# kowaalczyk/reformer-tts

Measured on AMD Instinct MI355X. Metric: mel-frames/sec training step, LJSpeech-shape batch, higher is better.
Workload: dtype bf16; 1 GPU; config/baseline.yml full Reformer-TTS training step (enc 3 / dec 3 layers, d=512, LSH 8 rounds, buckets 64/128), per-GPU batch 12, text 200->256, mel 1024x80; global_batch=12, parallelism=dp1, reversible_recompute=full

## Files before the change

### reformer-tts_amd/csrc/gemm_tn.hip

```cpp
#include "rtts_common.h"
#include <atomic>

#define GT_BM 64
#define GT_PAD 64

struct GtProb {
    const bf16_t* a;
    const bf16_t* b;
    float* out;
    float* c;
    int64_t lda, ldb, ldo, ldc;
    size_t slab_stride;
    int M, N, K, split, accumulate;
    int wg_start;
    int rb_start;
};
struct GtGroup {
    GtProb p[RTTS_GEMM_TN_MAX_GROUP];
    int n;
};

template <int WN, int WK, int TN, int TK>
__global__ __launch_bounds__(64 * WN * WK) void gemm_tn_kernel(const GtGroup grp) {
    constexpr int BN = 32 * TN * WN, BK = 32 * TK * WK, NTHR = 64 * WN * WK;
    constexpr int ROWA = BN * 2 + GT_PAD, ROWB = BK * 2 + GT_PAD;
    constexpr int PA = BN / 8, PB = BK / 8;
    constexpr int ITA = GT_BM * PA / NTHR, ITB = GT_BM * PB / NTHR;
    static_assert(GT_BM * PA % NTHR == 0 && GT_BM * PB % NTHR == 0, "staging must tile");
    extern __shared__ __attribute__((aligned(16))) unsigned char smem[];
    unsigned char* As = smem;
    unsigned char* Bs = smem + 2 * GT_BM * ROWA;

    int pi = 0;
#pragma unroll
    for (int i = 1; i < RTTS_GEMM_TN_MAX_GROUP; ++i)
        if (i < grp.n && (int)blockIdx.x >= grp.p[i].wg_start) pi = i;
    const GtProb& P = grp.p[pi];
    const bf16_t* __restrict__ a = P.a;
    const bf16_t* __restrict__ b = P.b;
    float* __restrict__ out = P.out;
    const int64_t lda = P.lda, ldb = P.ldb, ldo = P.ldo;
    const int M = P.M, K = P.K, split = P.split, accumulate = P.accumulate;
    const size_t slab_stride = P.slab_stride;
    const int blk = (int)blockIdx.x - P.wg_start;

    const int tiles_k = K / BK;
    const int tile = blk / split, sp = blk % split;
    const int n0 = (tile / tiles_k) * BN, k0 = (tile % tiles_k) * BK;
    const int st_all = M / GT_BM, st_base = st_all / split, st_rem = st_all % split;
    const int nstage = st_base + (sp < st_rem ? 1 : 0);
    const int m_begin = (sp * st_base + min(sp, st_rem)) * GT_BM;

    const int tid = threadIdx.x, lane = tid & 63, wave = tid >> 6;
    const int wn = wave / WK, wk = wave % WK;
    const int hh = lane >> 5;
    const int trq = (lane & 15) >> 2, trp = lane & 3, trc = (lane >> 4) & 1;

    const int arow = tid / PA, apiece = tid % PA, brow = tid / PB, bpiece = tid % PB;
    static_assert(ITA <= 4 && ITB <= 4, "staging registers");
    uint4 ra0, ra1, ra2, ra3, rb0, rb1, rb2, rb3;
#define GT_LD(reg, base, ld, step, it, IT) \
    if constexpr ((it) < (IT)) reg = *reinterpret_cast<const uint4*>((base) + (size_t)((it) * (step)) * (ld))
#define GT_ST(reg, base, bstep, it, IT) \
    if constexpr ((it) < (IT)) *reinterpret_cast<uint4*>((base) + (it) * (bstep)) = reg
#define GT_LOAD_STAGE(stage)                                                              \
    do {                                                                                  \
        const size_t m_ = (size_t)m_begin + (size_t)(stage) * GT_BM;                      \
        const bf16_t* pa_ = a + (m_ + arow) * lda + n0 + apiece * 8;                      \
        const bf16_t* pb_ = b + (m_ + brow) * ldb + k0 + bpiece * 8;                      \
        GT_LD(ra0, pa_, lda, NTHR / PA, 0, ITA); GT_LD(ra1, pa_, lda, NTHR / PA, 1, ITA); \
        GT_LD(ra2, pa_, lda, NTHR / PA, 2, ITA); GT_LD(ra3, pa_, lda, NTHR / PA, 3, ITA); \
        GT_LD(rb0, pb_, ldb, NTHR / PB, 0, ITB); GT_LD(rb1, pb_, ldb, NTHR / PB, 1, ITB); \
        GT_LD(rb2, pb_, ldb, NTHR / PB, 2, ITB); GT_LD(rb3, pb_, ldb, NTHR / PB, 3, ITB); \
    } while (0)
#define GT_STORE_STAGE(buf)                                                               \
    do {                                                                                  \
        unsigned char* pa_ = As + ((buf) * GT_BM + arow) * ROWA + apiece * 16;            \
        unsigned char* pb_ = Bs + ((buf) * GT_BM + brow) * ROWB + bpiece * 16;            \
        GT_ST(ra0, pa_, (NTHR / PA) * ROWA, 0, ITA); GT_ST(ra1, pa_, (NTHR / PA) * ROWA, 1, ITA); \
        GT_ST(ra2, pa_, (NTHR / PA) * ROWA, 2, ITA); GT_ST(ra3, pa_, (NTHR / PA) * ROWA, 3, ITA); \
        GT_ST(rb0, pb_, (NTHR / PB) * ROWB, 0, ITB); GT_ST(rb1, pb_, (NTHR / PB) * ROWB, 1, ITB); \
        GT_ST(rb2, pb_, (NTHR / PB) * ROWB, 2, ITB); GT_ST(rb3, pb_, (NTHR / PB) * ROWB, 3, ITB); \
    } while (0)

    f32x16 acc[TN][TK];
#pragma unroll
    for (int i = 0; i < TN; ++i)
#pragma unroll
        for (int j = 0; j < TK; ++j) acc[i][j] = (f32x16){0};

    GT_LOAD_STAGE(0);
    GT_STORE_STAGE(0);
    __syncthreads();
    for (int s = 0; s < nstage; ++s) {
        const int buf = s & 1;
        if (s + 1 < nstage) GT_LOAD_STAGE(s + 1);
        const unsigned char* Ab = As + buf * GT_BM * ROWA;
        const unsigned char* Bb = Bs + buf * GT_BM * ROWB;
#define GT_FRAGS(AF, BF, ks_)                                                                   \
    do {                                                                                        \
        const int mr_ = (ks_) * 16 + 8 * hh + trq;                                              \
        _Pragma("unroll") for (int t = 0; t < TN; ++t) {                                        \
            const int ca_ = (wn * 32 * TN + t * 32 + 16 * trc + 4 * trp) * 2;                   \
            AF[t] = rtts_tr_frag(Ab + mr_ * ROWA + ca_, Ab + (mr_ + 4) * ROWA + ca_);             \
        }                                                                                       \
        _Pragma("unroll") for (int t = 0; t < TK; ++t) {                                        \
            const int cb_ = (wk * 32 * TK + t * 32 + 16 * trc + 4 * trp) * 2;                   \
            BF[t] = rtts_tr_frag(Bb + mr_ * ROWB + cb_, Bb + (mr_ + 4) * ROWB + cb_);             \
        }                                                                                       \
    } while (0)
#define GT_MFMAS(AF, BF)                                                                        \
    _Pragma("unroll") for (int i = 0; i < TN; ++i)                                              \
        _Pragma("unroll") for (int j = 0; j < TK; ++j)                                          \
            acc[i][j] = __builtin_amdgcn_mfma_f32_32x32x16_bf16(AF[i], BF[j], acc[i][j], 0, 0, 0)
        bf16x8 af0[TN], bf0[TK], af1[TN], bf1[TK];
        GT_FRAGS(af0, bf0, 0);
        GT_FRAGS(af1, bf1, 1);
        __builtin_amdgcn_sched_barrier(0);
        GT_MFMAS(af0, bf0);
        __builtin_amdgcn_sched_barrier(0);
        GT_FRAGS(af0, bf0, 2);
        __builtin_amdgcn_sched_barrier(0);
        GT_MFMAS(af1, bf1);
        __builtin_amdgcn_sched_barrier(0);
        GT_FRAGS(af1, bf1, 3);
        __builtin_amdgcn_sched_barrier(0);
        GT_MFMAS(af0, bf0);
        __builtin_amdgcn_sched_barrier(0);
        GT_MFMAS(af1, bf1);
        static_assert(GT_BM == 64, "four k-steps per stage");
        if (s + 1 < nstage) GT_STORE_STAGE(buf ^ 1);
        __syncthreads();
    }
#undef GT_LOAD_STAGE
#undef GT_STORE_STAGE
#undef GT_LD
#undef GT_ST
#undef GT_FRAGS
#undef GT_MFMAS

    float* dst = out + (split > 1 ? (size_t)sp * slab_stride : 0);
    const bool add = (split == 1) && accumulate;
#pragma unroll
    for (int i = 0; i < TN; ++i)
#pragma unroll
        for (int j = 0; j < TK; ++j) {
            const int nb = n0 + wn * 32 * TN + i * 32 + 4 * hh;
            const int kc = k0 + wk * 32 * TK + j * 32 + (lane & 31);
#pragma unroll
            for (int e = 0; e < 16; ++e) {
                float* p = dst + (size_t)(nb + (e & 3) + 8 * (e >> 2)) * ldo + kc;
                *p = add ? *p + acc[i][j][e] : acc[i][j][e];
            }
        }
}

#define GT_RS 32
#define GT_NST 4

template <int WN, int WK, int TN, int TK>
__global__ __launch_bounds__(64 * WN * WK) void gemm_tn_ring_kernel(const GtGroup grp) {
    constexpr int BN = 32 * TN * WN, BK = 32 * TK * WK, NTHR = 64 * WN * WK, NWAVE = WN * WK;
    static_assert(BN == 256 && BK == 256 && NWAVE == 8, "ring variant: 256 x 256 tile, 8 waves");
    constexpr int ROWB = 512;
    constexpr int STAGE = GT_RS * ROWB;
    extern __shared__ __attribute__((aligned(16))) unsigned char smem[];
    unsigned char* As = smem;
    unsigned char* Bs = smem + GT_NST * STAGE;

    int pi = 0;
#pragma unroll
    for (int i = 1; i < RTTS_GEMM_TN_MAX_GROUP; ++i)
        if (i < grp.n && (int)blockIdx.x >= grp.p[i].wg_start) pi = i;
    const GtProb& P = grp.p[pi];
    const bf16_t* __restrict__ a = P.a;
    const bf16_t* __restrict__ b = P.b;
    float* __restrict__ out = P.out;
    const int64_t lda = P.lda, ldb = P.ldb, ldo = P.ldo;
    const int M = P.M, K = P.K, split = P.split, accumulate = P.accumulate;
    const size_t slab_stride = P.slab_stride;
    const int blk = (int)blockIdx.x - P.wg_start;
    const int tiles_k = K / BK;
    const int tile = blk / split, sp = blk % split;
    const int n0 = (tile / tiles_k) * BN, k0 = (tile % tiles_k) * BK;
    const int st_all = M / GT_RS, st_base = st_all / split, st_rem = st_all % split;
    const int nstage = st_base + (sp < st_rem ? 1 : 0);
    const int m_begin = (sp * st_base + min(sp, st_rem)) * GT_RS;

    const int tid = threadIdx.x, lane = tid & 63, wave = __builtin_amdgcn_readfirstlane(tid >> 6);
    const int wn = wave / WK, wk = wave % WK;
    const int hh = lane >> 5;
    const int trq = (lane & 15) >> 2, trp = lane & 3, trc = (lane >> 4) & 1;

    const bf16_t* srcA[2];
    const bf16_t* srcB[2];
#pragma unroll
    for (int i = 0; i < 2; ++i) {
        const int row = 4 * wave + 2 * i + (lane >> 5);
        const int pp = lane & 31;
        const int col = ((((pp >> 2) ^ (row & 3)) << 6) + ((pp & 3) << 4)) >> 1;
        srcA[i] = a + ((size_t)m_begin + row) * lda + n0 + col;
        srcB[i] = b + ((size_t)m_begin + row) * ldb + k0 + col;
    }
#define GT_ISSUE(stage_)                                                                                              \
    do {                                                                                                              \
        const int buf_ = (stage_) % GT_NST;                                                                           \
        const size_t mo_ = (size_t)(stage_) * GT_RS;                                                                  \
        _Pragma("unroll") for (int i = 0; i < 2; ++i) {                                                               \
            __builtin_amdgcn_global_load_lds((const __attribute__((address_space(1))) void*)(srcA[i] + mo_ * lda),    \
                                             (RTTS_LDS void*)(As + buf_ * STAGE + (4 * wave + 2 * i) * ROWB), 16, 0, 0); \
            __builtin_amdgcn_global_load_lds((const __attribute__((address_space(1))) void*)(srcB[i] + mo_ * ldb),    \
                                             (RTTS_LDS void*)(Bs + buf_ * STAGE + (4 * wave + 2 * i) * ROWB), 16, 0, 0); \
        }                                                                                                             \
    } while (0)

    f32x16 acc[TN][TK];
#pragma unroll
    for (int i = 0; i < TN; ++i)
#pragma unroll
        for (int j = 0; j < TK; ++j) acc[i][j] = (f32x16){0};

    int offA[TN], offB[TK];
#pragma unroll
    for (int t = 0; t < TN; ++t) {
        const int cb = (wn * 32 * TN + t * 32 + 16 * trc + 4 * trp) * 2;
        offA[t] = (8 * hh + trq) * ROWB + ((((cb >> 6) ^ trq) << 6) | (cb & 63));
    }
#pragma unroll
    for (int t = 0; t < TK; ++t) {
        const int cb = (wk * 32 * TK + t * 32 + 16 * trc + 4 * trp) * 2;
        offB[t] = (8 * hh + trq) * ROWB + ((((cb >> 6) ^ trq) << 6) | (cb & 63));
    }

    constexpr int AHEAD = GT_NST - 1;
    static_assert(AHEAD >= 2 && AHEAD <= 4, "ring depth 3..5");
#pragma unroll
    for (int i = 0; i < AHEAD; ++i)
        if (i < nstage) GT_ISSUE(i);
    for (int s = 0; s < nstage; ++s) {
        const int later = min(AHEAD - 1, nstage - 1 - s);
        if (later >= 3) __builtin_amdgcn_s_waitcnt(0x0F7C);
        else if (later == 2) __builtin_amdgcn_s_waitcnt(0x0F78);
        else if (later == 1) __builtin_amdgcn_s_waitcnt(0x0F74);
        else __builtin_amdgcn_s_waitcnt(0x0F70);
        asm volatile("s_barrier" ::: "memory");
        if (s + AHEAD < nstage) GT_ISSUE(s + AHEAD);
        const unsigned char* Ab = As + (s % GT_NST) * STAGE;
        const unsigned char* Bb = Bs + (s % GT_NST) * STAGE;
        const uint32_t abase = (uint32_t)(uintptr_t)(RTTS_LDS unsigned char*)Ab;
        const uint32_t bbase = (uint32_t)(uintptr_t)(RTTS_LDS unsigned char*)Bb;
        short4v al[2][TN], ah[2][TN], bl[2][TK], bh[2][TK];
#define GT_TR(dst, addr, off) asm volatile("ds_read_b64_tr_b16 %0, %1 offset:%2" : "=v"(dst) : "v"(addr), "n"(off))
#pragma unroll
        for (int t = 0; t < TN; ++t) {
            const uint32_t ad = abase + offA[t];
            GT_TR(al[0][t], ad, 0);
            GT_TR(ah[0][t], ad, 4 * ROWB);
            GT_TR(al[1][t], ad, 16 * ROWB);
            GT_TR(ah[1][t], ad, 20 * ROWB);
        }
#pragma unroll
        for (int t = 0; t < TK; ++t) {
            const uint32_t ad = bbase + offB[t];
            GT_TR(bl[0][t], ad, 0);
            GT_TR(bh[0][t], ad, 4 * ROWB);
            GT_TR(bl[1][t], ad, 16 * ROWB);
            GT_TR(bh[1][t], ad, 20 * ROWB);
        }
#undef GT_TR
        static_assert(TN == 2 && TK == 4, "operand list of the wait below");
        asm volatile("s_waitcnt lgkmcnt(0)"
                     : "+v"(al[0][0]), "+v"(ah[0][0]), "+v"(al[1][0]), "+v"(ah[1][0]), "+v"(al[0][1]), "+v"(ah[0][1]), "+v"(al[1][1]),
                       "+v"(ah[1][1]), "+v"(bl[0][0]), "+v"(bh[0][0]), "+v"(bl[1][0]), "+v"(bh[1][0]), "+v"(bl[0][1]), "+v"(bh[0][1]),
                       "+v"(bl[1][1]), "+v"(bh[1][1]), "+v"(bl[0][2]), "+v"(bh[0][2]), "+v"(bl[1][2]), "+v"(bh[1][2]), "+v"(bl[0][3]),
                       "+v"(bh[0][3]), "+v"(bl[1][3]), "+v"(bh[1][3]));
        bf16x8 af0[TN], bf0[TK], af1[TN], bf1[TK];
#pragma unroll
        for (int t = 0; t < TN; ++t) {
            const short8v f0 = {al[0][t][0], al[0][t][1], al[0][t][2], al[0][t][3], ah[0][t][0], ah[0][t][1], ah[0][t][2], ah[0][t][3]};
            const short8v f1 = {al[1][t][0], al[1][t][1], al[1][t][2], al[1][t][3], ah[1][t][0], ah[1][t][1], ah[1][t][2], ah[1][t][3]};
            af0[t] = __builtin_bit_cast(bf16x8, f0);
            af1[t] = __builtin_bit_cast(bf16x8, f1);
        }
#pragma unroll
        for (int t = 0; t < TK; ++t) {
            const short8v f0 = {bl[0][t][0], bl[0][t][1], bl[0][t][2], bl[0][t][3], bh[0][t][0], bh[0][t][1], bh[0][t][2], bh[0][t][3]};
            const short8v f1 = {bl[1][t][0], bl[1][t][1], bl[1][t][2], bl[1][t][3], bh[1][t][0], bh[1][t][1], bh[1][t][2], bh[1][t][3]};
            bf0[t] = __builtin_bit_cast(bf16x8, f0);
            bf1[t] = __builtin_bit_cast(bf16x8, f1);
        }
#pragma unroll
        for (int i = 0; i < TN; ++i)
#pragma unroll
            for (int j = 0; j < TK; ++j) acc[i][j] = __builtin_amdgcn_mfma_f32_32x32x16_bf16(af0[i], bf0[j], acc[i][j], 0, 0, 0);
#pragma unroll
        for (int i = 0; i < TN; ++i)
#pragma unroll
            for (int j = 0; j < TK; ++j) acc[i][j] = __builtin_amdgcn_mfma_f32_32x32x16_bf16(af1[i], bf1[j], acc[i][j], 0, 0, 0);
    }
#undef GT_ISSUE

    float* dst = out + (split > 1 ? (size_t)sp * slab_stride : 0);
    const bool add = (split == 1) && accumulate;
#pragma unroll
    for (int i = 0; i < TN; ++i)
#pragma unroll
        for (int j = 0; j < TK; ++j) {
            const int nb = n0 + wn * 32 * TN + i * 32 + 4 * hh;
            const int kc = k0 + wk * 32 * TK + j * 32 + (lane & 31);
#pragma unroll
            for (int e = 0; e < 16; ++e) {
                float* p = dst + (size_t)(nb + (e & 3) + 8 * (e >> 2)) * ldo + kc;
                *p = add ? *p + acc[i][j][e] : acc[i][j][e];
            }
        }
}

__global__ __launch_bounds__(256) void slab_reduce_kernel(const GtGroup grp) {
    int pi = 0;
#pragma unroll
    for (int i = 1; i < RTTS_GEMM_TN_MAX_GROUP; ++i)
        if (i < grp.n && (int)blockIdx.x >= grp.p[i].rb_start) pi = i;
    const GtProb& P = grp.p[pi];
    if (P.split == 1) return;
    const size_t i4 = (size_t)((int)blockIdx.x - P.rb_start) * blockDim.x + threadIdx.x;
    const size_t total4 = P.slab_stride / 4;
    if (i4 >= total4) return;
    const size_t e = i4 * 4;
    const int n = (int)(e / P.K), k = (int)(e % P.K);
    const float* __restrict__ slabs = P.out;
    float4 s = *reinterpret_cast<const float4*>(slabs + e);
    for (int t = 1; t < P.split; ++t) {
        const float4 v = *reinterpret_cast<const float4*>(slabs + (size_t)t * P.slab_stride + e);
        s.x += v.x; s.y += v.y; s.z += v.z; s.w += v.w;
    }
    float4* dst = reinterpret_cast<float4*>(P.c + (size_t)n * P.ldc + k);
    if (P.accumulate) {
        const float4 o = *dst;
        s.x += o.x; s.y += o.y; s.z += o.z; s.w += o.w;
    }
    *dst = s;
}

template <int WN, int WK, int TN, int TK>
static int gt_launch(const GtGroup& grp, int wg, hipStream_t s) {
    constexpr int BN = 32 * TN * WN, BK = 32 * TK * WK;
    const size_t lds = 2 * GT_BM * (BN * 2 + GT_PAD) + 2 * GT_BM * (BK * 2 + GT_PAD);
    static RttsLdsState st = {};
    RTTS_ENSURE_LDS("rtts_gemm_tn", (gemm_tn_kernel<WN, WK, TN, TK>), lds, st);
    hipLaunchKernelGGL((gemm_tn_kernel<WN, WK, TN, TK>), dim3(wg), dim3(64 * WN * WK), lds, s, grp);
    return 0;
}

static bool gt_c_overlap(const rtts_gemm_tn_problem& p, const rtts_gemm_tn_problem& q) {
    const uintptr_t bp = (uintptr_t)p.c, bq = (uintptr_t)q.c;
    const uintptr_t ep = bp + ((uintptr_t)(p.N - 1) * (uintptr_t)p.ldc + (uintptr_t)p.K) * sizeof(float);
    const uintptr_t eq = bq + ((uintptr_t)(q.N - 1) * (uintptr_t)q.ldc + (uintptr_t)q.K) * sizeof(float);
    if (bq >= ep || bp >= eq) return false;
    if (p.ldc != q.ldc) return true;
    const rtts_gemm_tn_problem& lo = bp <= bq ? p : q;
    const rtts_gemm_tn_problem& hi = bp <= bq ? q : p;
    const int64_t d = (int64_t)(((uintptr_t)hi.c - (uintptr_t)lo.c) / sizeof(float));
    const int64_t r = d / lo.ldc, s = d % lo.ldc;
    if (s < lo.K) return true;
    return s + hi.K > lo.ldc && r + 1 < lo.N;
}

static std::atomic<int> g_gt_small{0};
extern "C" int rtts_debug_set_gemm_tn_tiles(int small_tiles) {
    if (small_tiles != 0 && small_tiles != 1) {
        rtts_set_error("rtts_debug_set_gemm_tn_tiles: 0 (library's pick) or 1 (128 x 128 tiles for every group) (got %d)", small_tiles);
        return -1;
    }
    g_gt_small.store(small_tiles, std::memory_order_relaxed);
    return 0;
}

extern "C" int rtts_gemm_tn_grouped(const rtts_gemm_tn_problem* problems, int n, float* slab_ws, int64_t slab_ws_floats, void* stream) {
    RTTS_ENTER(stream);
    RTTS_REQUIRE(problems && n > 0 && n <= RTTS_GEMM_TN_MAX_GROUP, "rtts_gemm_tn_grouped: 1..%d problems", RTTS_GEMM_TN_MAX_GROUP);
    GtGroup grp;
    grp.n = n;
    bool big = g_gt_small.load(std::memory_order_relaxed) == 0;
    long long flops = 0;
    for (int i = 0; i < n; ++i) {
        const rtts_gemm_tn_problem& q = problems[i];
        RTTS_REQUIRE(q.a && q.b && q.c, "rtts_gemm_tn: null pointer");
        RTTS_REQUIRE(q.N > 0 && q.K > 0 && q.M > 0 && q.N % 128 == 0 && q.K % 128 == 0 && q.M % GT_BM == 0,
                     "rtts_gemm_tn: need N %% 128 == 0, K %% 128 == 0, M %% 64 == 0 (got M=%d N=%d K=%d)", q.M, q.N, q.K);
        RTTS_REQUIRE(q.lda >= q.N && q.ldb >= q.K && q.ldc >= q.K && q.lda % 8 == 0 && q.ldb % 8 == 0 && q.ldc % 4 == 0,
                     "rtts_gemm_tn: bad leading dimensions");
        RTTS_REQUIRE((((uintptr_t)q.a | (uintptr_t)q.b | (uintptr_t)q.c) & 15) == 0, "rtts_gemm_tn: buffers must be 16-byte aligned");
        big = big && q.N % 256 == 0 && q.K % 256 == 0;
        flops += 2LL * q.M * q.N * q.K;
    }
    for (int i = 1; i < n; ++i)
        for (int j = 0; j < i; ++j)
            RTTS_REQUIRE(!gt_c_overlap(problems[j], problems[i]),
                         "rtts_gemm_tn_grouped: problems %d and %d write overlapping parts of C (launch them one after the other)", j, i);
    if (flops < 40LL * 1000000000LL) big = false;
    const int bt = big ? 256 : 128;
    int total_tiles = 0;
    for (int i = 0; i < n; ++i) total_tiles += (problems[i].N / bt) * (problems[i].K / bt);
    const int wg_target = big ? 320 : 640;
    int want = 1;
    while (total_tiles * want * 2 <= wg_target) want *= 2;
    int wg = 0, rb = 0;
    size_t slab_used = 0;
    bool any_split = false;
    for (int i = 0; i < n; ++i) {
        const rtts_gemm_tn_problem& q = problems[i];
        GtProb& P = grp.p[i];
        const int tiles = (q.N / bt) * (q.K / bt), stages = q.M / GT_BM;
        const size_t slab = (size_t)q.N * q.K;
        int split = 1;
        while (split < want && split * 2 <= stages / 4) split *= 2;
        while (split > 1 && (!slab_ws || slab_used + slab * split > (size_t)slab_ws_floats)) split /= 2;
        P.a = (const bf16_t*)q.a; P.b = (const bf16_t*)q.b; P.c = q.c;
        P.lda = q.lda; P.ldb = q.ldb; P.ldc = q.ldc;
        P.M = q.M; P.N = q.N; P.K = q.K; P.split = split; P.accumulate = q.accumulate;
        P.slab_stride = slab;
        P.wg_start = wg;
        P.rb_start = rb;
        wg += tiles * split;
        if (split > 1) {
            P.out = slab_ws + slab_used;
            P.ldo = q.K;
            slab_used += slab * split;
            rb += (int)((slab / 4 + 255) / 256);
            any_split = true;
        } else {
            P.out = q.c;
            P.ldo = q.ldc;
        }
    }
    hipStream_t s = (hipStream_t)stream;
    if (big) {
        const size_t lds = 2 * GT_NST * GT_RS * 512;
        static RttsLdsState st = {};
        RTTS_ENSURE_LDS("rtts_gemm_tn", (gemm_tn_ring_kernel<4, 2, 2, 4>), lds, st);
        hipLaunchKernelGGL((gemm_tn_ring_kernel<4, 2, 2, 4>), dim3(wg), dim3(512), lds, s, grp);
    } else if (gt_launch<2, 2, 2, 2>(grp, wg, s)) return -1;
    if (any_split) hipLaunchKernelGGL(slab_reduce_kernel, dim3(rb), dim3(256), 0, s, grp);
    RTTS_LAUNCH_CHECK("rtts_gemm_tn");
    return 0;
}

extern "C" int rtts_gemm_tn(const void* a, int64_t lda, const void* b, int64_t ldb, int M, int N, int K, float* c, int64_t ldc,
                            int accumulate, float* slab_ws, int64_t slab_ws_floats, void* stream) {
    RTTS_ENTER(stream);
    rtts_gemm_tn_problem q;
    q.a = a; q.lda = lda; q.b = b; q.ldb = ldb; q.c = c; q.ldc = ldc;
    q.M = M; q.N = N; q.K = K; q.accumulate = accumulate;
    return rtts_gemm_tn_grouped(&q, 1, slab_ws, slab_ws_floats, stream);
}
```

Baseline: 1.999 million mel-frames/s.

## Unify TN GEMM on ring DMA kernel with software-pipelined LDS fragment reads

Removes the register-staged double-buffered small-tile kernel and routes small problems through the ring kernel, generalised to 128x128 tiles with direct global-to-LDS loads into a four-deep ring. The ring main loop is restructured to interleave transposed LDS fragment reads for the next half-step with MFMAs and DMA issues, using counted waits and one barrier per stage instead of reading everything and then computing. This aims to hide LDS read latency and global load latency behind matrix ops. Optional timestamp instrumentation is added behind a macro, and the hand-counted waitcnt logic makes correctness fragile.

```diff
diff --git a/reformer-tts_amd/csrc/gemm_tn.hip b/reformer-tts_amd/csrc/gemm_tn.hip
--- a/reformer-tts_amd/csrc/gemm_tn.hip
+++ b/reformer-tts_amd/csrc/gemm_tn.hip
@@ -1,8 +1,8 @@
 #include "rtts_common.h"
+#include "gemm_tn_tile.h"
 #include <atomic>
 
 #define GT_BM 64
-#define GT_PAD 64
 
 struct GtProb {
     const bf16_t* a;
@@ -20,150 +20,31 @@
     int n;
 };
 
-template <int WN, int WK, int TN, int TK>
-__global__ __launch_bounds__(64 * WN * WK) void gemm_tn_kernel(const GtGroup grp) {
-    constexpr int BN = 32 * TN * WN, BK = 32 * TK * WK, NTHR = 64 * WN * WK;
-    constexpr int ROWA = BN * 2 + GT_PAD, ROWB = BK * 2 + GT_PAD;
-    constexpr int PA = BN / 8, PB = BK / 8;
-    constexpr int ITA = GT_BM * PA / NTHR, ITB = GT_BM * PB / NTHR;
-    static_assert(GT_BM * PA % NTHR == 0 && GT_BM * PB % NTHR == 0, "staging must tile");
-    extern __shared__ __attribute__((aligned(16))) unsigned char smem[];
-    unsigned char* As = smem;
-    unsigned char* Bs = smem + 2 * GT_BM * ROWA;
-
-    int pi = 0;
-#pragma unroll
-    for (int i = 1; i < RTTS_GEMM_TN_MAX_GROUP; ++i)
-        if (i < grp.n && (int)blockIdx.x >= grp.p[i].wg_start) pi = i;
-    const GtProb& P = grp.p[pi];
-    const bf16_t* __restrict__ a = P.a;
-    const bf16_t* __restrict__ b = P.b;
-    float* __restrict__ out = P.out;
-    const int64_t lda = P.lda, ldb = P.ldb, ldo = P.ldo;
-    const int M = P.M, K = P.K, split = P.split, accumulate = P.accumulate;
-    const size_t slab_stride = P.slab_stride;
-    const int blk = (int)blockIdx.x - P.wg_start;
-
-    const int tiles_k = K / BK;
-    const int tile = blk / split, sp = blk % split;
-    const int n0 = (tile / tiles_k) * BN, k0 = (tile % tiles_k) * BK;
-    const int st_all = M / GT_BM, st_base = st_all / split, st_rem = st_all % split;
-    const int nstage = st_base + (sp < st_rem ? 1 : 0);
-    const int m_begin = (sp * st_base + min(sp, st_rem)) * GT_BM;
-
-    const int tid = threadIdx.x, lane = tid & 63, wave = tid >> 6;
-    const int wn = wave / WK, wk = wave % WK;
-    const int hh = lane >> 5;
-    const int trq = (lane & 15) >> 2, trp = lane & 3, trc = (lane >> 4) & 1;
-
-    const int arow = tid / PA, apiece = tid % PA, brow = tid / PB, bpiece = tid % PB;
-    static_assert(ITA <= 4 && ITB <= 4, "staging registers");
-    uint4 ra0, ra1, ra2, ra3, rb0, rb1, rb2, rb3;
-#define GT_LD(reg, base, ld, step, it, IT) \
-    if constexpr ((it) < (IT)) reg = *reinterpret_cast<const uint4*>((base) + (size_t)((it) * (step)) * (ld))
-#define GT_ST(reg, base, bstep, it, IT) \
-    if constexpr ((it) < (IT)) *reinterpret_cast<uint4*>((base) + (it) * (bstep)) = reg
-#define GT_LOAD_STAGE(stage)                                                              \
-    do {                                                                                  \
-        const size_t m_ = (size_t)m_begin + (size_t)(stage) * GT_BM;                      \
-        const bf16_t* pa_ = a + (m_ + arow) * lda + n0 + apiece * 8;                      \
-        const bf16_t* pb_ = b + (m_ + brow) * ldb + k0 + bpiece * 8;                      \
-        GT_LD(ra0, pa_, lda, NTHR / PA, 0, ITA); GT_LD(ra1, pa_, lda, NTHR / PA, 1, ITA); \
-        GT_LD(ra2, pa_, lda, NTHR / PA, 2, ITA); GT_LD(ra3, pa_, lda, NTHR / PA, 3, ITA); \
-        GT_LD(rb0, pb_, ldb, NTHR / PB, 0, ITB); GT_LD(rb1, pb_, ldb, NTHR / PB, 1, ITB); \
-        GT_LD(rb2, pb_, ldb, NTHR / PB, 2, ITB); GT_LD(rb3, pb_, ldb, NTHR / PB, 3, ITB); \
-    } while (0)
-#define GT_STORE_STAGE(buf)                                                               \
-    do {                                                                                  \
-        unsigned char* pa_ = As + ((buf) * GT_BM + arow) * ROWA + apiece * 16;            \
-        unsigned char* pb_ = Bs + ((buf) * GT_BM + brow) * ROWB + bpiece * 16;            \
-        GT_ST(ra0, pa_, (NTHR / PA) * ROWA, 0, ITA); GT_ST(ra1, pa_, (NTHR / PA) * ROWA, 1, ITA); \
-        GT_ST(ra2, pa_, (NTHR / PA) * ROWA, 2, ITA); GT_ST(ra3, pa_, (NTHR / PA) * ROWA, 3, ITA); \
-        GT_ST(rb0, pb_, (NTHR / PB) * ROWB, 0, ITB); GT_ST(rb1, pb_, (NTHR / PB) * ROWB, 1, ITB); \
-        GT_ST(rb2, pb_, (NTHR / PB) * ROWB, 2, ITB); GT_ST(rb3, pb_, (NTHR / PB) * ROWB, 3, ITB); \
-    } while (0)
-
-    f32x16 acc[TN][TK];
-#pragma unroll
-    for (int i = 0; i < TN; ++i)
-#pragma unroll
-        for (int j = 0; j < TK; ++j) acc[i][j] = (f32x16){0};
-
-    GT_LOAD_STAGE(0);
-    GT_STORE_STAGE(0);
-    __syncthreads();
-    for (int s = 0; s < nstage; ++s) {
-        const int buf = s & 1;
-        if (s + 1 < nstage) GT_LOAD_STAGE(s + 1);
-        const unsigned char* Ab = As + buf * GT_BM * ROWA;
-        const unsigned char* Bb = Bs + buf * GT_BM * ROWB;
-#define GT_FRAGS(AF, BF, ks_)                                                                   \
-    do {                                                                                        \
-        const int mr_ = (ks_) * 16 + 8 * hh + trq;                                              \
-        _Pragma("unroll") for (int t = 0; t < TN; ++t) {                                        \
-            const int ca_ = (wn * 32 * TN + t * 32 + 16 * trc + 4 * trp) * 2;                   \
-            AF[t] = rtts_tr_frag(Ab + mr_ * ROWA + ca_, Ab + (mr_ + 4) * ROWA + ca_);             \
-        }                                                                                       \
-        _Pragma("unroll") for (int t = 0; t < TK; ++t) {                                        \
-            const int cb_ = (wk * 32 * TK + t * 32 + 16 * trc + 4 * trp) * 2;                   \
-            BF[t] = rtts_tr_frag(Bb + mr_ * ROWB + cb_, Bb + (mr_ + 4) * ROWB + cb_);             \
-        }                                                                                       \
-    } while (0)
-#define GT_MFMAS(AF, BF)                                                                        \
-    _Pragma("unroll") for (int i = 0; i < TN; ++i)                                              \
-        _Pragma("unroll") for (int j = 0; j < TK; ++j)                                          \
-            acc[i][j] = __builtin_amdgcn_mfma_f32_32x32x16_bf16(AF[i], BF[j], acc[i][j], 0, 0, 0)
-        bf16x8 af0[TN], bf0[TK], af1[TN], bf1[TK];
-        GT_FRAGS(af0, bf0, 0);
-        GT_FRAGS(af1, bf1, 1);
-        __builtin_amdgcn_sched_barrier(0);
-        GT_MFMAS(af0, bf0);
-        __builtin_amdgcn_sched_barrier(0);
-        GT_FRAGS(af0, bf0, 2);
-        __builtin_amdgcn_sched_barrier(0);
-        GT_MFMAS(af1, bf1);
-        __builtin_amdgcn_sched_barrier(0);
-        GT_FRAGS(af1, bf1, 3);
-        __builtin_amdgcn_sched_barrier(0);
-        GT_MFMAS(af0, bf0);
-        __builtin_amdgcn_sched_barrier(0);
-        GT_MFMAS(af1, bf1);
-        static_assert(GT_BM == 64, "four k-steps per stage");
-        if (s + 1 < nstage) GT_STORE_STAGE(buf ^ 1);
-        __syncthreads();
-    }
-#undef GT_LOAD_STAGE
-#undef GT_STORE_STAGE
-#undef GT_LD
-#undef GT_ST
-#undef GT_FRAGS
-#undef GT_MFMAS
-
-    float* dst = out + (split > 1 ? (size_t)sp * slab_stride : 0);
-    const bool add = (split == 1) && accumulate;
-#pragma unroll
-    for (int i = 0; i < TN; ++i)
-#pragma unroll
-        for (int j = 0; j < TK; ++j) {
-            const int nb = n0 + wn * 32 * TN + i * 32 + 4 * hh;
-            const int kc = k0 + wk * 32 * TK + j * 32 + (lane & 31);
-#pragma unroll
-            for (int e = 0; e < 16; ++e) {
-                float* p = dst + (size_t)(nb + (e & 3) + 8 * (e >> 2)) * ldo + kc;
-                *p = add ? *p + acc[i][j][e] : acc[i][j][e];
-            }
-        }
-}
-
-#define GT_RS 32
+#define GT_RS GTT_RS
 #define GT_NST 4
+
+#ifdef GT_STAMPS
+__device__ unsigned long long g_gt_stamps[4 * 4096];
+extern "C" int rtts_debug_gt_stamps(void* dst) { return (int)hipMemcpyFromSymbol(dst, HIP_SYMBOL(g_gt_stamps), sizeof(g_gt_stamps)); }
+#define GT_STAMP(var) \
+    unsigned long long var; \
+    __builtin_amdgcn_sched_barrier(0); \
+    asm volatile("s_memtime %0\n\ts_waitcnt lgkmcnt(0)" : "=s"(var)::"memory"); \
+    __builtin_amdgcn_sched_barrier(0)
+#else
+#define GT_STAMP(var)
+#endif
 
 template <int WN, int WK, int TN, int TK>
 __global__ __launch_bounds__(64 * WN * WK) void gemm_tn_ring_kernel(const GtGroup grp) {
-    constexpr int BN = 32 * TN * WN, BK = 32 * TK * WK, NTHR = 64 * WN * WK, NWAVE = WN * WK;
-    static_assert(BN == 256 && BK == 256 && NWAVE == 8, "ring variant: 256 x 256 tile, 8 waves");
-    constexpr int ROWB = 512;
+    constexpr int BN = 32 * TN * WN, BK = 32 * TK * WK, NWAVE = WN * WK, NT = TN + TK, NMMA = TN * TK;
+    static_assert(BN == BK && (BN == 256 || BN == 128), "ring kernel: square tile of 256 or 128");
+    constexpr int ROWB = 2 * BN;
     constexpr int STAGE = GT_RS * ROWB;
+    constexpr int NDMA = STAGE / 1024 / NWAVE;
+    static_assert(NDMA == 2 && NDMA * NWAVE * 1024 == STAGE, "four DMA instructions per wave and stage (the vmcnt counts below)");
+    static_assert((NT == 6 && NMMA == 8) || (NT == 4 && NMMA == 4), "operand lists of the waits, MFMA sequence");
+    constexpr int UNIT = BN == 256 ? GT_RS : GT_BM;
     extern __shared__ __attribute__((aligned(16))) unsigned char smem[];
     unsigned char* As = smem;
     unsigned char* Bs = smem + GT_NST * STAGE;
@@ -183,22 +64,20 @@
     const int tiles_k = K / BK;
     const int tile = blk / split, sp = blk % split;
     const int n0 = (tile / tiles_k) * BN, k0 = (tile % tiles_k) * BK;
-    const int st_all = M / GT_RS, st_base = st_all / split, st_rem = st_all % split;
-    const int nstage = st_base + (sp < st_rem ? 1 : 0);
-    const int m_begin = (sp * st_base + min(sp, st_rem)) * GT_RS;
+    const int st_all = M / UNIT, st_base = st_all / split, st_rem = st_all % split;
+    const int nstage = (st_base + (sp < st_rem ? 1 : 0)) * (UNIT / GT_RS);
+    const int m_begin = (sp * st_base + min(sp, st_rem)) * UNIT;
 
     const int tid = threadIdx.x, lane = tid & 63, wave = __builtin_amdgcn_readfirstlane(tid >> 6);
     const int wn = wave / WK, wk = wave % WK;
     const int hh = lane >> 5;
-    const int trq = (lane & 15) >> 2, trp = lane & 3, trc = (lane >> 4) & 1;
-
-    const bf16_t* srcA[2];
-    const bf16_t* srcB[2];
-#pragma unroll
-    for (int i = 0; i < 2; ++i) {
-        const int row = 4 * wave + 2 * i + (lane >> 5);
-        const int pp = lane & 31;
-        const int col = ((((pp >> 2) ^ (row & 3)) << 6) + ((pp & 3) << 4)) >> 1;
+
+    const bf16_t* srcA[NDMA];
+    const bf16_t* srcB[NDMA];
+#pragma unroll
+    for (int i = 0; i < NDMA; ++i) {
+        const int row = gtt_dma_row<ROWB>(NDMA * wave + i, lane);
+        const int col = gtt_dma_src_col<ROWB>(NDMA * wave + i, lane) >> 1;
         srcA[i] = a + ((size_t)m_begin + row) * lda + n0 + col;
         srcB[i] = b + ((size_t)m_begin + row) * ldb + k0 + col;
     }
@@ -206,99 +85,124 @@
     do {                                                                                                              \
         const int buf_ = (stage_) % GT_NST;                                                                           \
         const size_t mo_ = (size_t)(stage_) * GT_RS;                                                                  \
-        _Pragma("unroll") for (int i = 0; i < 2; ++i) {                                                               \
+        _Pragma("unroll") for (int i = 0; i < NDMA; ++i) {                                                            \
             __builtin_amdgcn_global_load_lds((const __attribute__((address_space(1))) void*)(srcA[i] + mo_ * lda),    \
-                                             (RTTS_LDS void*)(As + buf_ * STAGE + (4 * wave + 2 * i) * ROWB), 16, 0, 0); \
+                                             (RTTS_LDS void*)(As + buf_ * STAGE + (NDMA * wave + i) * 1024), 16, 0, 0); \
             __builtin_amdgcn_global_load_lds((const __attribute__((address_space(1))) void*)(srcB[i] + mo_ * ldb),    \
-                                             (RTTS_LDS void*)(Bs + buf_ * STAGE + (4 * wave + 2 * i) * ROWB), 16, 0, 0); \
+                                             (RTTS_LDS void*)(Bs + buf_ * STAGE + (NDMA * wave + i) * 1024), 16, 0, 0); \
         }                                                                                                             \
     } while (0)
 
+#define GT_ISSUE1(stage_, q_)                                                                                         \
+    do {                                                                                                              \
+        const int buf_ = (stage_) % GT_NST;                                                                           \
+        const size_t mo_ = (size_t)(stage_) * GT_RS;                                                                  \
+        if constexpr (((q_) & 1) == 0)                                                                                \
+            __builtin_amdgcn_global_load_lds((const __attribute__((address_space(1))) void*)(srcA[(q_) >> 1] + mo_ * lda), \
+                                             (RTTS_LDS void*)(As + buf_ * STAGE + (NDMA * wave + ((q_) >> 1)) * 1024), 16, 0, 0); \
+        else                                                                                                          \
+            __builtin_amdgcn_global_load_lds((const __attribute__((address_space(1))) void*)(srcB[(q_) >> 1] + mo_ * ldb), \
+                                             (RTTS_LDS void*)(Bs + buf_ * STAGE + (NDMA * wave + ((q_) >> 1)) * 1024), 16, 0, 0); \
+    } while (0)
+
     f32x16 acc[TN][TK];
 #pragma unroll
     for (int i = 0; i < TN; ++i)
 #pragma unroll
         for (int j = 0; j < TK; ++j) acc[i][j] = (f32x16){0};
 
-    int offA[TN], offB[TK];
-#pragma unroll
-    for (int t = 0; t < TN; ++t) {
-        const int cb = (wn * 32 * TN + t * 32 + 16 * trc + 4 * trp) * 2;
-        offA[t] = (8 * hh + trq) * ROWB + ((((cb >> 6) ^ trq) << 6) | (cb & 63));
-    }
-#pragma unroll
-    for (int t = 0; t < TK; ++t) {
-        const int cb = (wk * 32 * TK + t * 32 + 16 * trc + 4 * trp) * 2;
-        offB[t] = (8 * hh + trq) * ROWB + ((((cb >> 6) ^ trq) << 6) | (cb & 63));
-    }
+    int off[NT];
+#pragma unroll
+    for (int t = 0; t < TN; ++t) off[t] = gtt_frag_off<ROWB>(wn * 32 * TN + t * 32, lane);
+#pragma unroll
+    for (int t = 0; t < TK; ++t) off[TN + t] = GT_NST * STAGE + gtt_frag_off<ROWB>(wk * 32 * TK + t * 32, lane);
 
     constexpr int AHEAD = GT_NST - 1;
-    static_assert(AHEAD >= 2 && AHEAD <= 4, "ring depth 3..5");
+    static_assert(AHEAD == 3, "the counted waits below");
+    short4v fl[2][NT], fh[2][NT];
+#define GT_TR(dst, addr, o_) asm volatile("ds_read_b64_tr_b16 %0, %1 offset:%2" : "=v"(dst) : "v"(addr), "n"(o_))
+#define GT_RD(h_, t_, base_)                                              \
+    do {                                                                  \
+        if constexpr ((t_) < NT) {                                        \
+            const uint32_t ad_ = (base_) + off[t_];                       \
+            GT_TR(fl[h_][t_], ad_, (16 * (h_)) * ROWB);                   \
+            GT_TR(fh[h_][t_], ad_, (16 * (h_) + 4) * ROWB);               \
+            __builtin_amdgcn_sched_barrier(0);                            \
+        }                                                                 \
+    } while (0)
+#define GT_WAIT(h_)                                                                                                          \
+    do {                                                                                                                     \
+        if constexpr (NT == 6)                                                                                               \
+            asm volatile("s_waitcnt lgkmcnt(0)"                                                                              \
+                         : "+v"(fl[h_][0]), "+v"(fh[h_][0]), "+v"(fl[h_][1]), "+v"(fh[h_][1]), "+v"(fl[h_][2]), "+v"(fh[h_][2]), \
+                           "+v"(fl[h_][3]), "+v"(fh[h_][3]), "+v"(fl[h_][NT - 2]), "+v"(fh[h_][NT - 2]), "+v"(fl[h_][NT - 1]),   \
+                           "+v"(fh[h_][NT - 1]));                                                                            \
+        else                                                                                                                 \
+            asm volatile("s_waitcnt lgkmcnt(0)"                                                                              \
+                         : "+v"(fl[h_][0]), "+v"(fh[h_][0]), "+v"(fl[h_][1]), "+v"(fh[h_][1]), "+v"(fl[h_][2]), "+v"(fh[h_][2]), \
+                           "+v"(fl[h_][3]), "+v"(fh[h_][3]));                                                                \
+        __builtin_amdgcn_sched_barrier(0);                                                                                   \
+    } while (0)
+#define GT_FRAG(h_, t_) \
+    __builtin_bit_cast(bf16x8, (short8v){fl[h_][t_][0], fl[h_][t_][1], fl[h_][t_][2], fl[h_][t_][3], fh[h_][t_][0], fh[h_][t_][1], fh[h_][t_][2], fh[h_][t_][3]})
+#define GT_STEP(h_, m_, g_, base_, dma_)                                                                                     \
+    do {                                                                                                                     \
+        GT_RD(g_, m_, base_);                                                                                                \
+        if constexpr ((m_) < NMMA) {                                                                                         \
+            acc[(m_) / TK][(m_) % TK] = __builtin_amdgcn_mfma_f32_32x32x16_bf16(GT_FRAG(h_, (m_) / TK), GT_FRAG(h_, TN + (m_) % TK), \
+                                                                              acc[(m_) / TK][(m_) % TK], 0, 0, 0);             \
+            __builtin_amdgcn_sched_barrier(0);                                                                               \
+        }                                                                                                                    \
+        if constexpr ((dma_) && (m_) < 2 * NDMA) {                                                                           \
+            if (more) GT_ISSUE1(s + AHEAD, m_);                                                                              \
+            __builtin_amdgcn_sched_barrier(0);                                                                               \
+        }                                                                                                                    \
+    } while (0)
+#define GT_HALF(h_, g_, base_, dma_)                                                                   \
+    do {                                                                                               \
+        GT_STEP(h_, 0, g_, base_, dma_); GT_STEP(h_, 1, g_, base_, dma_); GT_STEP(h_, 2, g_, base_, dma_); GT_STEP(h_, 3, g_, base_, dma_); \
+        GT_STEP(h_, 4, g_, base_, dma_); GT_STEP(h_, 5, g_, base_, dma_); GT_STEP(h_, 6, g_, base_, dma_); GT_STEP(h_, 7, g_, base_, dma_); \
+    } while (0)
+
+    const uint32_t ring = (uint32_t)(uintptr_t)(RTTS_LDS unsigned char*)As;
 #pragma unroll
     for (int i = 0; i < AHEAD; ++i)
         if (i < nstage) GT_ISSUE(i);
+    if (nstage >= 3) __builtin_amdgcn_s_waitcnt(0x0F78);
+    else if (nstage == 2) __builtin_amdgcn_s_waitcnt(0x0F74);
+    else __builtin_amdgcn_s_waitcnt(0x0F70);
+    asm volatile("s_barrier" ::: "memory");
+    __builtin_amdgcn_sched_barrier(0);
+    GT_RD(0, 0, ring); GT_RD(0, 1, ring); GT_RD(0, 2, ring); GT_RD(0, 3, ring); GT_RD(0, 4, ring); GT_RD(0, 5, ring);
+    GT_STAMP(t_loop0);
     for (int s = 0; s < nstage; ++s) {
-        const int later = min(AHEAD - 1, nstage - 1 - s);
-        if (later >= 3) __builtin_amdgcn_s_waitcnt(0x0F7C);
-        else if (later == 2) __builtin_amdgcn_s_waitcnt(0x0F78);
-        else if (later == 1) __builtin_amdgcn_s_waitcnt(0x0F74);
+        const uint32_t cur = ring + (s % GT_NST) * STAGE;
+        const uint32_t nxt = ring + ((s + 1 < nstage ? s + 1 : s) % GT_NST) * STAGE;
+        const bool more = s + AHEAD < nstage;
+        GT_WAIT(0);
+        GT_HALF(0, 1, cur, false);
+        if (s + 2 < nstage) __builtin_amdgcn_s_waitcnt(0x0F74);
         else __builtin_amdgcn_s_waitcnt(0x0F70);
         asm volatile("s_barrier" ::: "memory");
-        if (s + AHEAD < nstage) GT_ISSUE(s + AHEAD);
-        const unsigned char* Ab = As + (s % GT_NST) * STAGE;
-        const unsigned char* Bb = Bs + (s % GT_NST) * STAGE;
-        const uint32_t abase = (uint32_t)(uintptr_t)(RTTS_LDS unsigned char*)Ab;
-        const uint32_t bbase = (uint32_t)(uintptr_t)(RTTS_LDS unsigned char*)Bb;
-        short4v al[2][TN], ah[2][TN], bl[2][TK], bh[2][TK];
-#define GT_TR(dst, addr, off) asm volatile("ds_read_b64_tr_b16 %0, %1 offset:%2" : "=v"(dst) : "v"(addr), "n"(off))
-#pragma unroll
-        for (int t = 0; t < TN; ++t) {
-            const uint32_t ad = abase + offA[t];
-            GT_TR(al[0][t], ad, 0);
-            GT_TR(ah[0][t], ad, 4 * ROWB);
-            GT_TR(al[1][t], ad, 16 * ROWB);
-            GT_TR(ah[1][t], ad, 20 * ROWB);
-        }
-#pragma unroll
-        for (int t = 0; t < TK; ++t) {
-            const uint32_t ad = bbase + offB[t];
-            GT_TR(bl[0][t], ad, 0);
-            GT_TR(bh[0][t], ad, 4 * ROWB);
-            GT_TR(bl[1][t], ad, 16 * ROWB);
-            GT_TR(bh[1][t], ad, 20 * ROWB);
-        }
+        __builtin_amdgcn_sched_barrier(0);
+        GT_WAIT(1);
+        GT_HALF(1, 0, nxt, true);
+    }
+    GT_STAMP(t_loop1);
+#ifdef GT_STAMPS
+    if (tid == 0 && blockIdx.x < 4096) {
+        g_gt_stamps[4 * blockIdx.x + 0] = t_loop1 - t_loop0;
+        g_gt_stamps[4 * blockIdx.x + 1] = (unsigned long long)nstage;
+    }
+#endif
+#undef GT_ISSUE
+#undef GT_ISSUE1
 #undef GT_TR
-        static_assert(TN == 2 && TK == 4, "operand list of the wait below");
-        asm volatile("s_waitcnt lgkmcnt(0)"
-                     : "+v"(al[0][0]), "+v"(ah[0][0]), "+v"(al[1][0]), "+v"(ah[1][0]), "+v"(al[0][1]), "+v"(ah[0][1]), "+v"(al[1][1]),
-                       "+v"(ah[1][1]), "+v"(bl[0][0]), "+v"(bh[0][0]), "+v"(bl[1][0]), "+v"(bh[1][0]), "+v"(bl[0][1]), "+v"(bh[0][1]),
-                       "+v"(bl[1][1]), "+v"(bh[1][1]), "+v"(bl[0][2]), "+v"(bh[0][2]), "+v"(bl[1][2]), "+v"(bh[1][2]), "+v"(bl[0][3]),
-                       "+v"(bh[0][3]), "+v"(bl[1][3]), "+v"(bh[1][3]));
-        bf16x8 af0[TN], bf0[TK], af1[TN], bf1[TK];
-#pragma unroll
-        for (int t = 0; t < TN; ++t) {
-            const short8v f0 = {al[0][t][0], al[0][t][1], al[0][t][2], al[0][t][3], ah[0][t][0], ah[0][t][1], ah[0][t][2], ah[0][t][3]};
-            const short8v f1 = {al[1][t][0], al[1][t][1], al[1][t][2], al[1][t][3], ah[1][t][0], ah[1][t][1], ah[1][t][2], ah[1][t][3]};
-            af0[t] = __builtin_bit_cast(bf16x8, f0);
-            af1[t] = __builtin_bit_cast(bf16x8, f1);
-        }
-#pragma unroll
-        for (int t = 0; t < TK; ++t) {
-            const short8v f0 = {bl[0][t][0], bl[0][t][1], bl[0][t][2], bl[0][t][3], bh[0][t][0], bh[0][t][1], bh[0][t][2], bh[0][t][3]};
-            const short8v f1 = {bl[1][t][0], bl[1][t][1], bl[1][t][2], bl[1][t][3], bh[1][t][0], bh[1][t][1], bh[1][t][2], bh[1][t][3]};
-            bf0[t] = __builtin_bit_cast(bf16x8, f0);
-            bf1[t] = __builtin_bit_cast(bf16x8, f1);
-        }
-#pragma unroll
-        for (int i = 0; i < TN; ++i)
-#pragma unroll
-            for (int j = 0; j < TK; ++j) acc[i][j] = __builtin_amdgcn_mfma_f32_32x32x16_bf16(af0[i], bf0[j], acc[i][j], 0, 0, 0);
-#pragma unroll
-        for (int i = 0; i < TN; ++i)
-#pragma unroll
-            for (int j = 0; j < TK; ++j) acc[i][j] = __builtin_amdgcn_mfma_f32_32x32x16_bf16(af1[i], bf1[j], acc[i][j], 0, 0, 0);
-    }
-#undef GT_ISSUE
+#undef GT_RD
+#undef GT_WAIT
+#undef GT_FRAG
+#undef GT_STEP
+#undef GT_HALF
 
     float* dst = out + (split > 1 ? (size_t)sp * slab_stride : 0);
     const bool add = (split == 1) && accumulate;
@@ -343,12 +247,11 @@
 }
 
 template <int WN, int WK, int TN, int TK>
-static int gt_launch(const GtGroup& grp, int wg, hipStream_t s) {
-    constexpr int BN = 32 * TN * WN, BK = 32 * TK * WK;
-    const size_t lds = 2 * GT_BM * (BN * 2 + GT_PAD) + 2 * GT_BM * (BK * 2 + GT_PAD);
+static int gt_launch_ring(const GtGroup& grp, int wg, hipStream_t s) {
+    const size_t lds = 2 * GT_NST * GT_RS * (2 * 32 * TN * WN);
     static RttsLdsState st = {};
-    RTTS_ENSURE_LDS("rtts_gemm_tn", (gemm_tn_kernel<WN, WK, TN, TK>), lds, st);
-    hipLaunchKernelGGL((gemm_tn_kernel<WN, WK, TN, TK>), dim3(wg), dim3(64 * WN * WK), lds, s, grp);
+    RTTS_ENSURE_LDS("rtts_gemm_tn", (gemm_tn_ring_kernel<WN, WK, TN, TK>), lds, st);
+    hipLaunchKernelGGL((gemm_tn_ring_kernel<WN, WK, TN, TK>), dim3(wg), dim3(64 * WN * WK), lds, s, grp);
     return 0;
 }
 
@@ -436,11 +339,8 @@
     }
     hipStream_t s = (hipStream_t)stream;
     if (big) {
-        const size_t lds = 2 * GT_NST * GT_RS * 512;
-        static RttsLdsState st = {};
-        RTTS_ENSURE_LDS("rtts_gemm_tn", (gemm_tn_ring_kernel<4, 2, 2, 4>), lds, st);
-        hipLaunchKernelGGL((gemm_tn_ring_kernel<4, 2, 2, 4>), dim3(wg), dim3(512), lds, s, grp);
-    } else if (gt_launch<2, 2, 2, 2>(grp, wg, s)) return -1;
+        if (gt_launch_ring<4, 2, 2, 4>(grp, wg, s)) return -1;
+    } else if (gt_launch_ring<2, 2, 2, 2>(grp, wg, s)) return -1;
     if (any_split) hipLaunchKernelGGL(slab_reduce_kernel, dim3(rb), dim3(256), 0, s, grp);
     RTTS_LAUNCH_CHECK("rtts_gemm_tn");
     return 0;
diff --git a/reformer-tts_amd/csrc/gemm_tn_tile.h b/reformer-tts_amd/csrc/gemm_tn_tile.h
--- /dev/null
+++ b/reformer-tts_amd/csrc/gemm_tn_tile.h
@@ -0,0 +1,33 @@
+#pragma once
+
+#if defined(__HIPCC__) || defined(__CUDACC__)
+#define GTT_HD __host__ __device__
+#else
+#define GTT_HD
+#endif
+
+#define GTT_RS 32
+
+template <int ROWB>
+GTT_HD constexpr int gtt_off(int row, int cb) {
+    return row * ROWB + ((((cb >> 6) ^ (row & 3)) << 6) | (cb & 63));
+}
+
+template <int ROWB>
+GTT_HD constexpr int gtt_dma_row(int ins, int lane) { return ins * (1024 / ROWB) + lane / (ROWB / 16); }
+template <int ROWB>
+GTT_HD constexpr int gtt_dma_dst(int ins, int lane) { return ins * 1024 + lane * 16; }
+template <int ROWB>
+GTT_HD constexpr int gtt_dma_src_col(int ins, int lane) {
+    const int pp = lane % (ROWB / 16);
+    return (((pp >> 2) ^ (gtt_dma_row<ROWB>(ins, lane) & 3)) << 6) + ((pp & 3) << 4);
+}
+
+GTT_HD constexpr int gtt_frag_row(int lane) { return 8 * (lane >> 5) + ((lane & 15) >> 2); }
+GTT_HD constexpr int gtt_frag_col(int tcol, int lane) { return (tcol + 16 * ((lane >> 4) & 1) + 4 * (lane & 3)) * 2; }
+template <int ROWB>
+GTT_HD constexpr int gtt_frag_off(int tcol, int lane) { return gtt_off<ROWB>(gtt_frag_row(lane), gtt_frag_col(tcol, lane)); }
+
+static_assert(gtt_off<512>(5, 200) == 5 * 512 + ((3 ^ 1) << 6) + 8 && gtt_off<256>(6, 130) == 6 * 256 + 2, "images");
+static_assert(gtt_dma_row<512>(3, 40) == 7 && gtt_dma_row<256>(3, 40) == 14 && gtt_dma_src_col<256>(3, 40) == 0 && gtt_dma_src_col<512>(3, 40) == (1 << 6),
+              "DMA map");
```

Result: no change. 1.988 million mel-frames/s (-0.6%).
